# liuliu/ccv

Hardware: AMD Instinct MI355X
Metric: images/sec fwd+bwd VGG-D 224x224 bs256 (higher is better)
Workload: dtype f32 (Winograd-domain / fc GEMMs: exact bf16x3 split, all 9 products, fp32 accumulate); 1 GPU; VGG-D (ccv vgg_d_params, 225x225x3 crop, NHWC) forward+backward+SGD, batch 256 per GPU, random-init weights; global_batch=256, parallelism=dp1, conv_relu=convolution epilogue (NNC_MI355X_CONV_ALGO_FUSE_RELU)

## Files before the change

ccv_amd/csrc/cmd_conv.cpp:

```cpp
#include "gemm_launch.h"
#include "chan_sums.h"
#include "winograd.h"
#include "wino_fused.h"
#include "wino_wgrad_fused.h"
#include "conv_c3.h"
#include "conv_depthwise.h"

using namespace nnc;

namespace {

static size_t align256(size_t x) { return (x + 255) & ~(size_t)255; }

struct back_share_t {
	int want_v;
	int want_bits;
	int GYn, GXn, KB;
	float* v;
	unsigned* bits;
	size_t v_off, bits_off;
};

static void* g_dbg_bits_dst = 0;
static size_t g_dbg_bits_cap = 0, g_dbg_bits_got = 0;
static long g_back_shared[2] = { 0, 0 };

struct conv_geom_t {
	int N, H, W, C;
	int OH, OW, K;
	int kh, kw, Cg, Kg, groups;
	int sy, sx, pby, pbx, dy, dx;
};

struct conv_call_t {
	int relu_want, relu_done, mask_want, mask_done;
	Image4 mask;
	int staged;
	back_share_t share;
};
static bool mask_fits(const Image4& m, const Image4& dst)
// ... 159 lines not shown
	const long TH = (g.H + 3) / 4, TW = (g.W + 3) / 4;
	long most = 0;
	static const int shapes[3][2] = { { 4, 4 }, { 2, 8 }, { 8, 2 } };
	for (int i = 0; i < 3; i++) {
		const long cover = ((TH + shapes[i][0] - 1) / shapes[i][0]) * ((TW + shapes[i][1] - 1) / shapes[i][1]);
		if (cover > most) most = cover;
	}
	return (size_t)g.N * most * ((g.C + WF_KT - 1) / WF_KT) * 1024;
}

template <bool FLIP>
static int conv_wino_fused_run(conv_call_t& call, const char* name, const conv_geom_t& g, const wino_fused_plan_t& p, const Image4& src, const float* w, const float* bias, const Image4& dst, const int pad_y, const int pad_x, ccv_nnc_stream_context_t* const ctx)
{
	const back_share_t& share = call.share;
	size_t bits_bytes = FLIP && mask_fits(call.mask, dst) && (long)p.groups * p.KB <= 0x7fffffffL ? (size_t)p.groups * p.KB * 1024 : 0;
	bool have_bits = FLIP && bits_bytes && share.bits && p.GH == 2 && p.GYn == share.GYn && p.GXn == share.GXn && p.KB == share.KB && p.uf_bytes <= share.bits_off;
	float* UF = (float*)workspace_of(ctx, have_bits ? share.bits_off + bits_bytes : p.uf_bytes + bits_bytes);
	if (have_bits && (!UF || (unsigned*)((char*)UF + share.bits_off) != share.bits)) { have_bits = false; UF = (float*)workspace_of(ctx, p.uf_bytes + bits_bytes); }
	if (!UF && bits_bytes) { bits_bytes = 0; UF = (float*)workspace_of(ctx, p.uf_bytes); }
	if (!UF) return CCV_NNC_EXEC_OOM;
	hipStream_t stream = stream_of(ctx);
	unsigned* const bits = have_bits ? share.bits : (bits_bytes ? (unsigned*)((char*)UF + p.uf_bytes) : 0);
	if (have_bits) call.mask_done = 1;
	else if (bits) {
		const dim3 grid((unsigned)((long)p.groups * p.KB));
		const Image4& m = call.mask;
		if (p.GH == 4) hipLaunchKernelGGL(HIP_KERNEL_NAME(wino_mask_pack_kernel<4, 4>), grid, dim3(256), 0, stream, (const float*)m.p, m.sn, m.sh, m.sw, bits, dst.h, dst.w, dst.c, p.GYn, p.GXn, p.KB);
		else if (p.GH == 2) hipLaunchKernelGGL(HIP_KERNEL_NAME(wino_mask_pack_kernel<2, 8>), grid, dim3(256), 0, stream, (const float*)m.p, m.sn, m.sh, m.sw, bits, dst.h, dst.w, dst.c, p.GYn, p.GXn, p.KB);
		else hipLaunchKernelGGL(HIP_KERNEL_NAME(wino_mask_pack_kernel<8, 2>), grid, dim3(256), 0, stream, (const float*)m.p, m.sn, m.sh, m.sw, bits, dst.h, dst.w, dst.c, p.GYn, p.GXn, p.KB);
		HIP_ENFORCE(hipGetLastError());
		call.mask_done = 1;
	}
	if (bits && g_dbg_bits_dst) {
		g_dbg_bits_got = (size_t)p.groups * p.KB * 1024;
		HIP_ENFORCE(hipMemcpyAsync(g_dbg_bits_dst, bits, g_dbg_bits_got < g_dbg_bits_cap ? g_dbg_bits_got : g_dbg_bits_cap, hipMemcpyDeviceToHost, stream));
		HIP_ENFORCE(hipStreamSynchronize(stream));
		g_dbg_bits_dst = 0;
	}
// ... 89 lines not shown
	if (bits && (share.GYn * 2 != p.t.TH || share.GXn * 8 != p.t.TW || g.C % WF_KT)) {
		const int r = fill_f32((float*)bits, bits_bytes / sizeof(float), 0.f, ctx);
		if (r != CCV_NNC_EXEC_SUCCESS) return r;
	}
	for (int n0 = 0; n0 < g.N; n0 += nb) {
		const int ns = g.N - n0 < nb ? g.N - n0 : nb;
		const int T = ns * per_image;
		WinoTiles ti;
		ti.TH = p.t.TH; ti.TW = p.t.TW; ti.T = T;
		ti.H = a.h; ti.W = a.w; ti.sn = a.sn; ti.sh = a.sh; ti.sw = a.sw; ti.oy = -g.pby; ti.ox = -g.pbx; ti.C4 = g.C / 4;
		ti.d_c4.init(ti.C4); ti.d_tw.init(ti.TW); ti.d_th.init(ti.TH);
		if (bits) {
			WinoMaskOut mo;
			mo.bits = (unsigned char*)bits; mo.GYn = share.GYn; mo.GXn = share.GXn; mo.KB = share.KB;
			hipLaunchKernelGGL(HIP_KERNEL_NAME(wino_input_kernel<true>), dim3(blocks_exact((size_t)T * ti.C4, 256)), dim3(256), 0, stream, (const float*)a.p + (long)n0 * a.sn, V, ti, mo);
			share.bits = bits; share.bits_off = p.total();
			__atomic_fetch_add(&g_back_shared[1], 1L, __ATOMIC_RELAXED);
		} else hipLaunchKernelGGL(HIP_KERNEL_NAME(wino_input_kernel<false>), dim3(blocks_exact((size_t)T * ti.C4, 256)), dim3(256), 0, stream, (const float*)a.p + (long)n0 * a.sn, V, ti, WinoMaskOut());
		HIP_ENFORCE(hipGetLastError());
		ti.H = gr.h; ti.W = gr.w; ti.sn = gr.sn; ti.sh = gr.sh; ti.sw = gr.sw; ti.oy = 0; ti.ox = 0; ti.C4 = g.K / 4;
		ti.d_c4.init(ti.C4);
		const long blocks = ((long)T * (g.K / 4) + 255) / 256;
		const float* const grs = (const float*)gr.p + (long)n0 * gr.sn;
		if (Vg) {
			ti.oy = -1; ti.ox = -1;
			hipLaunchKernelGGL(wino_outgrad_both_kernel, dim3((unsigned)blocks), dim3(256), 0, stream, grs, Vg, W, ti, BP);
			share.v = Vg; share.v_off = p.total();
			__atomic_fetch_add(&g_back_shared[0], 1L, __ATOMIC_RELAXED);
		} else if (fuse_bias) hipLaunchKernelGGL(HIP_KERNEL_NAME(wino_outgrad_kernel<true>), dim3((unsigned)blocks), dim3(256), 0, stream, grs, W, ti, BP);
		else hipLaunchKernelGGL(HIP_KERNEL_NAME(wino_outgrad_kernel<false>), dim3((unsigned)blocks), dim3(256), 0, stream, grs, W, ti, (float*)0);
		HIP_ENFORCE(hipGetLastError());
// ... 44 lines not shown
	p->partial_bytes = (sizeof(float) * 36 * (size_t)s * g.K * g.C + 255) & ~(size_t)255;
	p->bias_bytes = (sizeof(float) * 4 * (size_t)s * g.K + 255) & ~(size_t)255;
	p->du_bytes = (sizeof(float) * 36 * (size_t)g.K * g.C + 255) & ~(size_t)255;
	return true;
}
static bool wino_wgrad_fused_images_ok(const Image4& a, const Image4& gr, const float* dw)
{
	const auto ok = [](const Image4& t) { return t.sc == 1 && aligned16(t.p) && t.sw % 4 == 0 && t.sh % 4 == 0 && (t.n == 1 || t.sn % 4 == 0) && ((long)(t.h - 1) * t.sh + (long)(t.w - 1) * t.sw + t.c) * 4 < 0x7ffff000L; };
	return ok(a) && ok(gr) && dw != 0;
}
static bool wino_wgrad_fused_preferred(const conv_geom_t& g)
{
	const long m = tune(TUNE_WINO_WGRAD_FUSED_MAX);
	return m > 0 && g.C <= m && g.K <= m;
}
static int conv_wino_wgrad_fused(const conv_geom_t& g, const wino_wgrad_fused_plan_t& p, const Image4& gr, const Image4& a, float* dw, float* dbias, bool* bias_done, const int flags, ccv_nnc_stream_context_t* const ctx)
{
	char* const ws = (char*)workspace_of(ctx, p.total());
	if (!ws) return CCV_NNC_EXEC_OOM;
	hipStream_t stream = stream_of(ctx);
	WinoWgradFusedArgs k;
	k.a = a.p; k.g = gr.p; k.partial = (float*)ws; k.bias_partial = dbias ? (float*)(ws + p.partial_bytes) : 0;
	k.a_sn = a.sn; k.a_sh = a.sh; k.a_sw = a.sw; k.g_sn = gr.sn; k.g_sh = gr.sh; k.g_sw = gr.sw;
	k.H = a.h; k.W = a.w; k.OH = gr.h; k.OW = gr.w; k.pad_y = g.pby; k.pad_x = g.pbx;
	k.GYn = p.GYn; k.GXn = p.GXn; k.groups = p.groups; k.C = g.C; k.K = g.K; k.kblocks = p.kblocks; k.cblocks = p.cblocks;
	k.slices = p.slices; k.per_slice = p.per_slice;
	k.a_image_bytes = (unsigned)(((long)(a.h - 1) * a.sh + (long)(a.w - 1) * a.sw + a.c) * 4);
	k.g_image_bytes = (unsigned)(((long)(gr.h - 1) * gr.sh + (long)(gr.w - 1) * gr.sw + gr.c) * 4);
	note_kernel("conv_wgrad_wino_fused");
	{
		const long T = (long)g.N * p.TH * p.TW;
		ProfScope prof("conv_wgrad_wino_fused|nnc::wino_wgrad_fused_kernel", 2.0 * 36.0 * (double)T * g.K * g.C, 0, g.K, g.C, (int)T, 36, p.slices, stream);
		hipLaunchKernelGGL(HIP_KERNEL_NAME(wino_wgrad_fused_kernel<0>), dim3((unsigned)(p.slices * p.kblocks * p.cblocks)), dim3(256), 0, stream, k);
		HIP_ENFORCE(hipGetLastError());
	}
	const long n = 36L * g.K * g.C;
	const int acc = (flags & CCV_NNC_ACCUMULATE_OUTPUT) ? 1 : 0;
	float* const dU = (float*)(ws + p.partial_bytes + p.bias_bytes);
	hipLaunchKernelGGL(wino_wgrad_fused_fold_kernel, dim3(blocks_exact((size_t)n, 256)), dim3(256), 0, stream, (const float*)k.partial, (const float*)k.bias_partial, dU, dbias, n, g.K, p.slices, acc);
	HIP_ENFORCE(hipGetLastError());
	hipLaunchKernelGGL(wino_wgrad_final_kernel, dim3(blocks_exact((size_t)g.K * g.C, 256)), dim3(256), 0, stream, (const float*)dU, dw, g.K, g.C, acc);
	HIP_ENFORCE(hipGetLastError());
	if (bias_done) *bias_done = dbias != 0;
	return CCV_NNC_EXEC_SUCCESS;
}

static bool wino_images_ok(const Image4& src, const Image4& dst, const float* w, const float* bias)
{
// ... 248 lines not shown
{
	return algo != CONV_ALGO_IMPLICIT_GEMM && wino_wgrad_plan(g, wp) && wino_images_ok(a, gr, dw, 0) && (algo >= CONV_ALGO_WINOGRAD || wino_preferred(wp->t, g.C, g.K));
}

static int conv_wgrad_nhwc(conv_call_t& call, const conv_geom_t& g, const Image4& gr, const Image4& a, float* dw, float* dbias, bool* bias_done, const int algo, const int flags, ccv_nnc_stream_context_t* const ctx)
{
	if (bias_done) *bias_done = false;
	if (a.sc != 1 || !pixel_linear(gr) || !image_fits_int(a)) return CCV_NNC_EXEC_INVALID;
	if (algo != CONV_ALGO_IMPLICIT_GEMM && conv_c3_ok(g, a, gr)) {
		const int r = conv_c3_wgrad(g, gr, a, dw, dbias, flags, ctx);
		if (r == CCV_NNC_EXEC_SUCCESS && bias_done) *bias_done = dbias != 0;
		if (r != CCV_NNC_EXEC_OOM) return r;
	}
	wino_wgrad_fused_plan_t wfp;
	if (conv_wgrad_takes_fused(g, gr, a, dw, algo, &wfp)) {
		const int r = conv_wino_wgrad_fused(g, wfp, gr, a, dw, dbias, bias_done, flags, ctx);
		if (r != CCV_NNC_EXEC_OOM) return r;
	}
	wino_wgrad_plan_t wp;
	if (conv_wgrad_takes_wino(g, gr, a, dw, algo, &wp)) {
		const int r = conv_wino_wgrad(call, g, wp, gr, a, dw, dbias, bias_done, flags, ctx);
		if (r != CCV_NNC_EXEC_OOM) return r;
	}
	const long P = (long)g.N * g.OH * g.OW;
	if (P > 0x7fffffffL) return CCV_NNC_EXEC_INVALID;
	const int NN = g.kh * g.kw * g.Cg;
	const bool vec = (g.Cg % 4 == 0) && (g.Kg % 4 == 0) && aligned16(a.p) && aligned16(gr.p) && a.sw % 4 == 0 && a.sh % 4 == 0 && (a.n == 1 || a.sn % 4 == 0) && gr.sw % 4 == 0;
	GemmOut out = { dw, (long)NN, 1, 0, 1.f, (flags & CCV_NNC_ACCUMULATE_OUTPUT) ? 1 : 0 };
	if (vec && conv_pointwise(g, a, gr)) {
		MatLoader<false, true> la, lb;
		la.p = gr.p; la.ldr = 1; la.ldk = gr.sw; la.R = g.K; la.K = (int)P;
// ... 438 lines not shown
	wino_wgrad_plan_t wgp;
	if (dw && cmd.algorithm != CONV_ALGO_IMPLICIT_GEMM && wino_wgrad_plan(g, &wgp) && wgp.total() > inner) inner = wgp.total();
	wino_wgrad_fused_plan_t wfgp;
	if (dw && cmd.algorithm != CONV_ALGO_IMPLICIT_GEMM && wino_wgrad_fused_plan(g, &wfgp) && wfgp.total() > inner) inner = wfgp.total();
	if (h && cmd.algorithm != CONV_ALGO_IMPLICIT_GEMM && wino_fused_scratch_bound(g.C, g.K) + wino_fused_mask_bound(call, g) > inner) inner = wino_fused_scratch_bound(g.C, g.K) + wino_fused_mask_bound(call, g);
	if (h && cmd.algorithm != CONV_ALGO_IMPLICIT_GEMM && conv_dgrad_parity_scratch(g) > inner) inner = conv_dgrad_parity_scratch(g);
	if (dw && cmd.algorithm != CONV_ALGO_IMPLICIT_GEMM && g.C == 3 && conv_c3_wgrad_scratch_bound(g.K) > inner) inner = conv_c3_wgrad_scratch_bound(g.K);
	back_share_t& share = call.share = back_share_t();
	const long share_on = tune(TUNE_CONV_BACK_SHARE);
	if (h && dw && a && w && share_on && !stage_io && !stage_w && g.pby == 1 && g.pbx == 1 && g.OH == g.H && g.OW == g.W && ai.sc == 1 && gi.sc == 1 && pixel_linear(gi) && pixel_linear(hi) && image_fits_int(ai) && image_fits_int(gi)
		&& !(cmd.algorithm != CONV_ALGO_IMPLICIT_GEMM && conv_c3_ok(g, ai, gi))) {
		wino_wgrad_fused_plan_t wf;
		wino_wgrad_plan_t wg;
		wino_fused_plan_t fp;
		wino_plan_t wp;
		if (!conv_wgrad_takes_fused(g, gi, ai, dw->data.f32, cmd.algorithm, &wf) && conv_wgrad_takes_wino(g, gi, ai, dw->data.f32, cmd.algorithm, &wg) && wino_slice_images(g.N, wg.t.TH * wg.t.TW, g.C, g.K) == g.N) {
			if (conv_dgrad_takes_fused(g, gi, hi, cmd.algorithm, &fp)) {
				if ((share_on & 2) && call.mask_want && fp.GH == 2 && mask_fits(ai, hi) && (long)fp.groups * fp.KB <= 0x7fffffffL && fp.uf_bytes <= wg.total()) {
					share.want_bits = 1; share.GYn = fp.GYn; share.GXn = fp.GXn; share.KB = fp.KB;
					if (wg.total() + (size_t)fp.groups * fp.KB * 1024 > inner) inner = wg.total() + (size_t)fp.groups * fp.KB * 1024;
				}
			} else if ((share_on & 1) && dbias && 256 % (g.K / 4) == 0 && conv_dgrad_takes_wino(g, gi, w->data.f32, hi, cmd.algorithm, &wp) && wp.TH == wg.t.TH && wp.TW == wg.t.TW && wp.u_bytes + wp.m_bytes <= wg.total()) {
				share.want_v = 1;
				if (wg.total() + wg.w_bytes > inner) inner = wg.total() + wg.w_bytes;
			}
		}
	}
	WorkspaceScope ws(stream_context, ng + na + nh + nw + ndw, inner);
	char* p = (char*)ws.prefix();
	if ((ng + na + nh + nw + ndw) && !p) return CCV_NNC_EXEC_OOM;
	int ret;
// ... 494 lines not shown
			const int ret = fwd ? _conv_forw(call, c, hint, trial_flags, inputs, input_size, outputs, output_size, stream_context) : _conv_back(call, c, hint, trial_flags, inputs, input_size, outputs, output_size, stream_context);
			HIP_ENFORCE(hipEventRecord(e1, stream));
			HIP_ENFORCE(hipEventSynchronize(e1));
			if (ret != CCV_NNC_EXEC_SUCCESS) ok = 0;
			else HIP_ENFORCE(hipEventElapsedTime(&ms, e0, e1));
		}
		if (ok && (!have_best || ms < best_ms)) { best = algo; best_ms = ms; have_best = 1; }
	}
	HIP_ENFORCE(hipEventDestroy(e0));
	HIP_ENFORCE(hipEventDestroy(e1));
	return best;
}

}

extern "C" long nnc_mi355x_debug_conv_back_shared(int what) { return what == 0 || what == 1 ? __atomic_load_n(&g_back_shared[what], __ATOMIC_RELAXED) : 0; }
extern "C" size_t nnc_mi355x_debug_conv_mask_bits(void* dst, size_t capacity)
{
	g_dbg_bits_dst = dst; g_dbg_bits_cap = capacity;
	return g_dbg_bits_got;
}

extern "C" void _register_command_CCV_NNC_CONVOLUTION_FORWARD_backend_CCV_NNC_BACKEND_GPU_CUDNN(ccv_nnc_cmd_backend_registry_t* const registry)
{
	registry->tensor_formats = CCV_TENSOR_FORMAT_NCHW | CCV_TENSOR_FORMAT_NHWC;
	registry->tensor_datatypes = CCV_32F | CCV_16F;
	registry->tensor_memory = CCV_TENSOR_GPU_MEMORY;
	registry->algorithms = CONV_ALGO_COUNT;
	registry->exec = _conv_forw_any;
	registry->autotune = _conv_autotune;
	NNC_DEPALETTIZED(registry, _conv_forw_any);
// ... 24 lines not shown
```

ccv_amd/csrc/device_rt.cpp:

```cpp
#include "common.h"
#include <atomic>
#include <pthread.h>
#include <dlfcn.h>
#include <vector>
#include <list>
#include <deque>
#include <mutex>
#include <unordered_map>

namespace {

struct device_local_t {
	hipStream_t stream;
	void* workspace;
	size_t workspace_size;
	int device;
	void* staging;
	size_t staging_size;
	void* palette;
	size_t palette_size;
	void* cluster_sync;
	unsigned cluster_epoch;
	unsigned long cluster_capture;
	unsigned long capture_alias;
// ... 91 lines not shown
	return l;
}

inline hipStream_t effective_stream(device_local_t* const l)
{
	if (g_capture_active.load(std::memory_order_acquire) > 0 && l->capture_alias == g_capture_id.load(std::memory_order_acquire) && l->capture_alias && l->device >= 0 && l->device < CAP_MAX_DEVICES && g_cap_rep[l->device]) return g_cap_rep[l->device];
	return l->stream;
}

}

namespace nnc {
int g_force_tile = 0;
int g_force_splits = 0;
static const char* const g_tune_names[TUNE_COUNT] = { "WINO_SLICE_KB", "WINO_FUSED_MAX_C", "WINO_FUSED_GRID", "GRID_WG_PER_CU", "WINO_WGRAD_FUSED_MAX", "GEMM_BUFFER_LOADS", "CONV_NCHW_HALF_F16", "BN_SMALL_PLANES", "SDPA_MFMA", "BN_CLUSTER", "GEMM_VEC_EPILOGUE", "POOL_ROWS", "GEMM_HALF_CHUNK8", "LSTM_PERSISTENT", "LSTM_ROWS", "GEMM_BF16X3", "BN_CLUSTER_SLOTS", "GEMM_BATCH_XCD", "CONV_BACK_SHARE", "CONV_DEPTHWISE", "ACT_HALF_NATIVE", "MUL_PLANES" };
static long g_tune_values[TUNE_COUNT] = { 0, 128, 0, 0, 128, 1, 32, 1, 1, 1, 1, 1, 1, 1, 1, 1, 0, 1, 3, 1, 1, 1 };
static int g_tune_env_read = 0;
long tune(int key)
{
	if (!g_tune_env_read) {
		for (int i = 0; i < TUNE_COUNT; i++) {
			char name[64];
			snprintf(name, sizeof(name), "NNC_MI355X_%s", g_tune_names[i]);
			const char* v = getenv(name);
			if (v && *v) g_tune_values[i] = atol(v);
		}
		g_tune_env_read = 1;
	}
	return key >= 0 && key < TUNE_COUNT ? g_tune_values[key] : 0;
}
}
// ... 1234 lines not shown
```

ccv_amd/csrc/isa.h:

```cpp
#pragma once
#include <hip/hip_runtime.h>

namespace nnc {

typedef float floatx16 __attribute__((ext_vector_type(16)));
typedef float floatx4 __attribute__((ext_vector_type(4)));
typedef _Float16 half_t;
typedef _Float16 halfx8 __attribute__((ext_vector_type(8)));
typedef _Float16 halfx4 __attribute__((ext_vector_type(4)));
typedef int wf_rsrc_t __attribute__((ext_vector_type(4)));
typedef unsigned int bf16x8_t __attribute__((ext_vector_type(4)));

#ifdef NNC_HIP_EMULATOR

#define NNC_PIN_V(x) ((void)0)
#define NNC_PIN_S(x) ((void)0)
#define WF_WAIT_VMCNT(n) __builtin_amdgcn_wave_barrier()
#define WF_MFMA(ACC, A, B, IN_AGPR) (ACC) = __builtin_amdgcn_mfma_f32_16x16x4f32((A), (B), (ACC), 0, 0, 0)
#define WF_MFMA0(ACC, A, B, IN_AGPR) (ACC) = __builtin_amdgcn_mfma_f32_16x16x4f32((A), (B), (floatx4{ 0.f, 0.f, 0.f, 0.f }), 0, 0, 0)
__device__ __forceinline__ wf_rsrc_t wf_make_rsrc(const void* base, unsigned bytes)
{
	const unsigned long long b = (unsigned long long)base;
	return wf_rsrc_t{ (int)(unsigned)b, (int)(unsigned)(b >> 32), (int)bytes, 0 };
}
__device__ __forceinline__ unsigned wf_lds_addr(float* p) { return (unsigned)(unsigned long long)p; }
__device__ __forceinline__ void wf_dma16(const wf_rsrc_t r, float* lds_base, unsigned lds_addr, unsigned voff, unsigned soff)
{
	const unsigned long long b = (unsigned long long)(unsigned)r[0] | (unsigned long long)(unsigned)r[1] << 32;
	float* const dst = (float*)((char*)lds_base + (lds_addr - wf_lds_addr(lds_base)));
// ... 20 lines not shown
#define NNC_PK_FMA_HI(acc, h, rp) do { (acc)[0] += (h)[0] * (rp)[1]; (acc)[1] += (h)[1] * (rp)[1]; } while (0)
#define NNC_WAIT_VM0_ONLY() ((void)0)
static inline float nnc_fast_exp2(const float x) { return exp2f(x); }
static inline float nnc_fast_rcp(const float x) { return 1.f / x; }
#define NNC_LAUNCH_CONCURRENT(kernel, grid, block, shmem, stream, ...) emuLaunchConcurrentKernel(kernel, grid, block, shmem, stream, __VA_ARGS__)
static inline unsigned nnc_fetch_add_agent(unsigned* p, unsigned v) { const unsigned o = *p; *p = o + v; return o; }
static inline void nnc_store_agent(unsigned* p, unsigned v) { *p = v; }
static inline void nnc_store_granule(unsigned long long* p, unsigned tag, float value) { unsigned u; memcpy(&u, &value, 4); *p = ((unsigned long long)tag << 32) | u; }
static inline unsigned long long nnc_load_granule(const unsigned long long* p) { return *(const volatile unsigned long long*)p; }
#define NNC_SPIN_SLEEP() emu::spin_yield()
static inline unsigned nnc_mul24(unsigned a, unsigned b) { return (a & 0xffffffu) * (b & 0xffffffu); }

#else

__device__ __forceinline__ unsigned nnc_mul24(unsigned a, unsigned b) { return __umul24(a, b); }

#define NNC_PIN_V(x) asm volatile("" : "+v"(x))
#define NNC_PIN_S(x) asm volatile("" : "+s"(x))
#define WF_WAIT_VMCNT(n) __builtin_amdgcn_s_waitcnt(((n) & 15) | (7 << 4) | (15 << 8) | (((n) >> 4) << 14))
#define WF_MFMA0(ACC, A, B, IN_AGPR) do { \
		if (IN_AGPR) asm volatile("v_mfma_f32_16x16x4_f32 %0, %1, %2, 0" : "+a"(ACC) : "v"(A), "v"(B)); \
		else asm volatile("v_mfma_f32_16x16x4_f32 %0, %1, %2, 0" : "+v"(ACC) : "v"(A), "v"(B)); \
	} while (0)
#define WF_MFMA(ACC, A, B, IN_AGPR) do { \
		if (IN_AGPR) asm volatile("v_mfma_f32_16x16x4_f32 %0, %1, %2, %0" : "+a"(ACC) : "v"(A), "v"(B)); \
		else asm volatile("v_mfma_f32_16x16x4_f32 %0, %1, %2, %0" : "+v"(ACC) : "v"(A), "v"(B)); \
	} while (0)
__device__ __forceinline__ wf_rsrc_t wf_make_rsrc(const void* base, unsigned bytes)
{
	const unsigned long long b = (unsigned long long)base;
// ... 53 lines not shown
```

ccv_amd/csrc/wino_fused.h:

```cpp
#pragma once
#include <utility>
#include "winograd.h"

namespace nnc {

constexpr int WF_KT = 32;
constexpr int WF_CC = 8;
constexpr int WF_U_FLOATS = 36 * 64 * 2 * 2;
constexpr int WF_HP = 352;
constexpr int WF_P_FLOATS = 2 * WF_HP * 4;
constexpr int WF_P_PIECES = 11;
constexpr int WF_Z_AGPR = 30;
constexpr unsigned WF_OOB = 0x7ffff000u;

template <class F, int... I> __device__ __forceinline__ void wf_static_for_impl(F&& f, std::integer_sequence<int, I...>) { (f(GroupId<I>()), ...); }
template <int N, class F> __device__ __forceinline__ void wf_static_for(F&& f) { wf_static_for_impl(f, std::make_integer_sequence<int, N>()); }

typedef float f2 __attribute__((ext_vector_type(2)));

template <int GH, int GW>
struct WfGeom {
	static constexpr int RH = 4 * GH + 2, RW = 4 * GW + 2, NPIX = RH * RW;
	static_assert(GH * GW == 16 && NPIX <= WF_HP, "tile group must be 16 tiles whose patch region fits the buffer");
	static constexpr __host__ __device__ int cy(int yy) { return GH + (yy < 2 ? 1 : 0); }
// ... 330 lines not shown
		const __amdgpu_buffer_rsrc_t rs_dst = __builtin_amdgcn_make_buffer_rsrc((void*)(a.dst + (long)it.n * a.d_sn), 0, a.dst_image_bytes, 0x00020000);
		const int kq = it.kb * WF_KT + (lane & 7) * 4;
		const bool kok = (it.live != 0) & (kq < a.K);
		float bv[4];
#pragma unroll
		for (int i = 0; i < 4; i++) bv[i] = (a.bias && kq < a.K) ? a.bias[kq + i] : 0.f;
		const int dh4 = (int)a.d_sh * 4, dw4 = (int)a.d_sw * 4;
		const wf_rsrc_t rs_item = wf_make_rsrc(a.dst + (long)it.n * a.d_sn, a.dst_image_bytes);
		const int base_y = it.gy * GH * 4, base_x = it.gx * GW * 4;
		const unsigned s_item = (unsigned)base_y * (unsigned)dh4 + (unsigned)base_x * (unsigned)dw4 + (unsigned)it.kb * (WF_KT * 4);
		const int hy0 = a.OH - base_y, hx0 = a.OW - base_x;
		const int ly = lane >> 5, lx = (lane >> 3) & 3;
		const unsigned lane_off_item = kok ? (unsigned)(ly * dh4 + lx * dw4 + (lane & 7) * 16) : WF_OOB;
		const float relu_lo = a.relu ? 0.f : -__builtin_inff();
		unsigned mb[4] = { ~0u, ~0u, ~0u, ~0u };
		if constexpr (MASK) {
			const unsigned* const mp = a.mask_bits + ((((long)it.n * a.GYn + it.gy) * a.GXn + it.gx) * a.KB + it.kb) * 256 + lane;
#pragma unroll
			for (int r = 0; r < 4; r++) mb[r] = it.live ? mp[r * 64] : 0u;
		}
#pragma unroll
		for (int r = 0; r < 4; r++) {
#pragma unroll
			for (int j = 0; j < 2; j++) {
				float s[4][6];
				if constexpr (DBG & 2048) {
#pragma unroll
					for (int i = 0; i < 4; i++)
#pragma unroll
						for (int jj = 0; jj < 4; jj++) st[g * TS + (i * 4 + jj) * 32 + j * 16 + ti] = acc[i * 4 + jj][j][r];
					continue;
// ... 5 lines not shown
					wino_at(col, y);
#pragma unroll
					for (int i = 0; i < 4; i++) s[i][zx] = y[i];
				}
#pragma unroll
				for (int i = 0; i < 4; i++) {
					float y[4];
					wino_at(s[i], y);
#pragma unroll
					for (int jj = 0; jj < 4; jj++) st[g * TS + (i * 4 + jj) * 32 + j * 16 + ti] = y[jj];
				}
			}
			__builtin_amdgcn_wave_barrier();
			if (r == 0) WF_WAIT_VMCNT(0);
			if constexpr (NEWST) {
#pragma unroll
				for (int e = 0; e < 8; e++) {
					const int tile = 4 * (e >> 1) + r;
					const int cy = (tile >> GWL) * 4 + (e & 1) * 2, cx = (tile & (GW - 1)) * 4;
					const float4 v = *(const float4*)(st + (e >> 1) * TS + ((e & 1) * 8 + (lane >> 3)) * 32 + (lane & 7) * 4);
					const unsigned soff = s_item + (unsigned)cy * (unsigned)dh4 + (unsigned)cx * (unsigned)dw4;
					const bool ok = (ly < hy0 - cy) & (lx < hx0 - cx);
					const unsigned voff = ok ? lane_off_item : WF_OOB;
					float o0 = wf_max(v.x + bv[0], relu_lo), o1 = wf_max(v.y + bv[1], relu_lo), o2 = wf_max(v.z + bv[2], relu_lo), o3 = wf_max(v.w + bv[3], relu_lo);
					if constexpr (MASK) {
						const unsigned m = mb[r] >> (4 * e);
						o0 = (m & 1) ? o0 : 0.f; o1 = (m & 2) ? o1 : 0.f; o2 = (m & 4) ? o2 : 0.f; o3 = (m & 8) ? o3 : 0.f;
					}
					if constexpr (DBG & 128) { NNC_PIN_V(o0); NNC_PIN_V(o1); NNC_PIN_V(o2); NNC_PIN_V(o3); }
					else wf_store16<ST_POLICY>(rs_item, voff, soff, o0, o1, o2, o3);
				}
			} else {
#pragma unroll
			for (int e = 0; e < 8; e++) {
				const int pid = e * 8 + (lane >> 3);
				const int gp = pid >> 4, px = pid & 15;
				const int tile = 4 * gp + r;
				const int oy = (it.gy * GH + (tile >> GWL)) * 4 + (px >> 2), ox = (it.gx * GW + (tile & (GW - 1))) * 4 + (px & 3);
				const float4 v = *(const float4*)(st + gp * TS + px * 32 + (lane & 7) * 4);
				const unsigned voff = (kok & (oy < a.OH) & (ox < a.OW)) ? (unsigned)(oy * dh4 + ox * dw4 + kq * 4) : WF_OOB;
// ... 88 lines not shown
```

ccv_amd/csrc/wino_wgrad_fused.h:

```cpp
#pragma once
#include "wino_fused.h"

namespace nnc {

typedef float f2v __attribute__((ext_vector_type(2)));

constexpr int WG_KB = 32, WG_CB = 64;
constexpr int WG_GH = 2, WG_GW = 4;
constexpr int WG_RH = 4 * WG_GH + 2, WG_RW = 4 * WG_GW + 2;
constexpr int WG_A_BYTES = WG_RH * WG_RW * WG_CB * 4;
constexpr int WG_G_BYTES = (4 * WG_GH) * (4 * WG_GW) * WG_KB * 4;
constexpr int WG_A_PIECES = WG_A_BYTES / 1024, WG_G_PIECES = WG_G_BYTES / 1024;
constexpr int WG_STAGE_BYTES = WG_A_BYTES + WG_G_BYTES;
static_assert(WG_A_BYTES % 1024 == 0 && WG_G_BYTES % 1024 == 0 && 2 * WG_STAGE_BYTES <= 160 * 1024, "two stages of whole DMA pieces in LDS");
constexpr int WG_A_PER_WAVE = (WG_A_PIECES + 3) / 4, WG_G_PER_WAVE = WG_G_PIECES / 4;
constexpr int WG_PIECES_PER_WAVE = WG_A_PER_WAVE + WG_G_PER_WAVE;

struct WinoWgradFusedArgs {
	const float* a;
	const float* g;
	float* partial;
	float* bias_partial;
	long a_sn, a_sh, a_sw, g_sn, g_sh, g_sw;
	int H, W, OH, OW;
	int pad_y, pad_x;
	int GYn, GXn;
	int groups;
	int C, K;
	int kblocks, cblocks;
	int slices;
	int per_slice;
	unsigned a_image_bytes, g_image_bytes;
};

template <int DBG = 0>
__global__ void __launch_bounds__(256, 1) wino_wgrad_fused_kernel(const WinoWgradFusedArgs p)
{
	__shared__ __attribute__((aligned(16))) float lds[2 * WG_STAGE_BYTES / 4 + 256];
	const int t = threadIdx.x, lane = t & 63;
	const int wave = __builtin_amdgcn_readfirstlane(t >> 6) & 3;
	const int wk = wave >> 1, wc = wave & 1;
	const int ch = lane & 15, slot = lane >> 4;
	const int nb = p.kblocks * p.cblocks;
	const int xcd = (int)blockIdx.x & 7, r = (int)blockIdx.x >> 3;
	const int slice = xcd * (p.slices >> 3) + r / nb, blk = r % nb;
	const int kb = blk / p.cblocks, cb = blk - kb * p.cblocks;
	int g_first = slice * p.per_slice, g_end = g_first + p.per_slice;
	if (g_end > p.groups) g_end = p.groups;
	const int gpi = p.GYn * p.GXn;

// ... 7 lines not shown
	int ayx[WG_A_PER_WAVE], gyx[WG_G_PER_WAVE];
#pragma unroll
	for (int i = 0; i < WG_A_PER_WAVE; i++) {
		const int q = wave + 4 * i, pi = q * 4 + (lane >> 4);
		ayx[i] = q < WG_A_PIECES ? ((pi / WG_RW) << 8 | (pi % WG_RW)) : 0xff00;
	}
#pragma unroll
	for (int i = 0; i < WG_G_PER_WAVE; i++) {
		const int pj = (wave + 4 * i) * 8 + (lane >> 3);
		gyx[i] = (pj / (4 * WG_GW)) << 8 | (pj % (4 * WG_GW));
	}
	const int a_coff = (cb * WG_CB + (lane & 15) * 4) * 4, g_coff = (kb * WG_KB + (lane & 7) * 4) * 4;
	const int a_sh4 = (int)p.a_sh * 4, a_sw4 = (int)p.a_sw * 4, g_sh4 = (int)p.g_sh * 4, g_sw4 = (int)p.g_sw * 4;
	const unsigned lds0 = __builtin_amdgcn_readfirstlane(wf_lds_addr(lds));
	wf_rsrc_t rs_a, rs_g;
	int aY0 = 0, aY1 = 0, aX0 = 0, aX1 = 0, gY1 = 0, gX1 = 0;
	auto set_group = [&](const int group) {
		const int n = group / gpi, gr = group - n * gpi;
		const int gy = gr / p.GXn, gx = gr - gy * p.GXn;
		const int ny0 = gy * 4 * WG_GH, nx0 = gx * 4 * WG_GW, nY0 = ny0 - p.pad_y, nX0 = nx0 - p.pad_x;
		rs_a = wf_make_rsrc(p.a + (long)n * p.a_sn + (long)nY0 * p.a_sh + (long)nX0 * p.a_sw, 0x7fff0000u);
		rs_g = wf_make_rsrc(p.g + (long)n * p.g_sn + (long)ny0 * p.g_sh + (long)nx0 * p.g_sw, 0x7fff0000u);
		aY0 = nY0 < 0 ? -nY0 : 0; aY1 = p.H - nY0 < WG_RH ? p.H - nY0 : WG_RH;
		aX0 = nX0 < 0 ? -nX0 : 0; aX1 = p.W - nX0 < WG_RW ? p.W - nX0 : WG_RW;
		gY1 = p.OH - ny0 < 4 * WG_GH ? p.OH - ny0 : 4 * WG_GH;
		gX1 = p.OW - nx0 < 4 * WG_GW ? p.OW - nx0 : 4 * WG_GW;
	};
	auto dma_piece = [&](auto ic, const int st, const bool live) {
		constexpr int i = decltype(ic)::value;
		if constexpr (i < WG_A_PER_WAVE) {
			const int Y = ayx[i] >> 8, X = ayx[i] & 255;
			const bool ok = live & (Y >= aY0) & (Y < aY1) & (X >= aX0) & (X < aX1);
			const unsigned voff = ok ? (unsigned)(Y * a_sh4 + X * a_sw4 + a_coff) : WF_OOB;
			const unsigned dst = wave + 4 * i < WG_A_PIECES ? lds0 + st * WG_STAGE_BYTES + (wave + 4 * i) * 1024 : lds0 + 2 * WG_STAGE_BYTES;
			wf_dma16(rs_a, lds, dst, voff, 0u);
		} else {
			constexpr int j = i - WG_A_PER_WAVE;
			const int y = gyx[j] >> 8, x = gyx[j] & 255;
			const bool ok = live & (y < gY1) & (x < gX1);
			const unsigned voff = ok ? (unsigned)(y * g_sh4 + x * g_sw4 + g_coff) : WF_OOB;
			wf_dma16(rs_g, lds, lds0 + st * WG_STAGE_BYTES + WG_A_BYTES + (wave + 4 * j) * 1024, voff, 0u);
		}
	};

	if (g_first < g_end) {
	set_group(g_first);
	NNC_ASM_NOPS("s_nop 4");
	wf_static_for<WG_PIECES_PER_WAVE>([&](auto nc) {
		constexpr int n = decltype(nc)::value, piece = n < 7 ? n : (n < 11 ? WG_A_PER_WAVE + (n - 7) : n - 4);
		dma_piece(GroupId<piece>(), 0, true);
	});

	for (int grp = g_first; grp < g_end; grp++) {
		const int st = (grp - g_first) & 1;
		if constexpr (!(DBG & 32)) {
			WF_WAIT_VMCNT(5);
			__builtin_amdgcn_s_barrier();
		}
		const bool has_next = grp + 1 < g_end;
		if (has_next) set_group(grp + 1);
		const float* const ab = lds + st * (WG_STAGE_BYTES / 4) + (4 * slot) * WG_CB + wc * 32 + 2 * ch;
		const float* const gb = lds + st * (WG_STAGE_BYTES / 4) + WG_A_BYTES / 4 + (4 * slot) * WG_KB + wk * 16 + ch;
		f2v W[36];
		if constexpr (DBG & 2) {
#pragma unroll
			for (int z = 0; z < 36; z++) W[z] = f2v{ 1.f + z, 2.f };
		} else {
			f2v e[4][4];
#pragma unroll
			for (int i = 0; i < 4; i++)
#pragma unroll
				for (int j = 0; j < 4; j++) e[i][j] = f2v{ gb[(i * (4 * WG_GW) + j) * WG_KB], gb[((4 + i) * (4 * WG_GW) + j) * WG_KB] };
// ... 56 lines not shown
				constexpr int mm = decltype(mc)::value, z = mm >> 1, jf = mm & 1;
				if constexpr (!(DBG & 16)) {
					if constexpr (ks == 0 && jf == 0) WF_MFMA(acc[z][0], W[z].x, V[z].x, z < WF_Z_AGPR);
					else if constexpr (ks == 0) WF_MFMA(acc[z][1], W[z].x, V[z].y, z < WF_Z_AGPR);
					else if constexpr (jf == 0) WF_MFMA(acc[z][0], W[z].y, V[z].x, z < WF_Z_AGPR);
					else WF_MFMA(acc[z][1], W[z].y, V[z].y, z < WF_Z_AGPR);
				}
				constexpr int m = ks * 72 + mm;
				if constexpr (m % 9 == 0 && !(DBG & 1)) {
					constexpr int n = m / 9;
					constexpr int piece = n < 7 ? n : (n < 11 ? WG_A_PER_WAVE + (n - 7) : n - 4);
					dma_piece(GroupId<piece>(), st ^ 1, has_next);
				}
			});
		});
	}
	}

	NNC_ASM_NOPS("s_nop 15\n\ts_nop 15");
	{
		float* const out = p.partial + (long)slice * 36 * p.K * p.C + (long)(kb * WG_KB + wk * 16 + 4 * slot) * p.C + cb * WG_CB + wc * 32 + 2 * ch;
		const long plane = (long)p.K * p.C;
#pragma unroll
		for (int z = 0; z < 36; z++)
#pragma unroll
			for (int j = 0; j < 2; j++)
#pragma unroll
				for (int i = 0; i < 4; i++) out[z * plane + (long)i * p.C + j] = acc[z][j][i];
		if (p.bias_partial && wc == 0 && cb == 0) p.bias_partial[((long)slice * 4 + slot) * p.K + kb * WG_KB + wk * 16 + ch] = bsum;
	}
// ... 24 lines not shown
```

Measured before the change: 3310 images/s.

## Emit ReLU mask bits from fused Winograd wgrad kernel for dgrad reuse

Result: no change. 3319 images/s, median of 5 (+0.3%).

```diff
diff --git a/ccv_amd/csrc/cmd_conv.cpp b/ccv_amd/csrc/cmd_conv.cpp
--- a/ccv_amd/csrc/cmd_conv.cpp
+++ b/ccv_amd/csrc/cmd_conv.cpp
@@ -15,15 +15,17 @@
 struct back_share_t {
 	int want_v;
 	int want_bits;
+	int want_bits_fused;
 	int GYn, GXn, KB;
 	float* v;
 	unsigned* bits;
+	int bits_gh;
 	size_t v_off, bits_off;
 };
 
 static void* g_dbg_bits_dst = 0;
 static size_t g_dbg_bits_cap = 0, g_dbg_bits_got = 0;
-static long g_back_shared[2] = { 0, 0 };
+static long g_back_shared[4] = { 0, 0, 0, 0 };
 
 struct conv_geom_t {
 	int N, H, W, C;
@@ -213,14 +215,14 @@
 {
 	const back_share_t& share = call.share;
 	size_t bits_bytes = FLIP && mask_fits(call.mask, dst) && (long)p.groups * p.KB <= 0x7fffffffL ? (size_t)p.groups * p.KB * 1024 : 0;
-	bool have_bits = FLIP && bits_bytes && share.bits && p.GH == 2 && p.GYn == share.GYn && p.GXn == share.GXn && p.KB == share.KB && p.uf_bytes <= share.bits_off;
+	bool have_bits = FLIP && bits_bytes && share.bits && p.GH == share.bits_gh && p.GYn == share.GYn && p.GXn == share.GXn && p.KB == share.KB && p.uf_bytes <= share.bits_off;
 	float* UF = (float*)workspace_of(ctx, have_bits ? share.bits_off + bits_bytes : p.uf_bytes + bits_bytes);
 	if (have_bits && (!UF || (unsigned*)((char*)UF + share.bits_off) != share.bits)) { have_bits = false; UF = (float*)workspace_of(ctx, p.uf_bytes + bits_bytes); }
 	if (!UF && bits_bytes) { bits_bytes = 0; UF = (float*)workspace_of(ctx, p.uf_bytes); }
 	if (!UF) return CCV_NNC_EXEC_OOM;
 	hipStream_t stream = stream_of(ctx);
 	unsigned* const bits = have_bits ? share.bits : (bits_bytes ? (unsigned*)((char*)UF + p.uf_bytes) : 0);
-	if (have_bits) call.mask_done = 1;
+	if (have_bits) { call.mask_done = 1; __atomic_fetch_add(&g_back_shared[3], 1L, __ATOMIC_RELAXED); }
 	else if (bits) {
 		const dim3 grid((unsigned)((long)p.groups * p.KB));
 		const Image4& m = call.mask;
@@ -340,7 +342,7 @@
 			WinoMaskOut mo;
 			mo.bits = (unsigned char*)bits; mo.GYn = share.GYn; mo.GXn = share.GXn; mo.KB = share.KB;
 			hipLaunchKernelGGL(HIP_KERNEL_NAME(wino_input_kernel<true>), dim3(blocks_exact((size_t)T * ti.C4, 256)), dim3(256), 0, stream, (const float*)a.p + (long)n0 * a.sn, V, ti, mo);
-			share.bits = bits; share.bits_off = p.total();
+			share.bits = bits; share.bits_off = p.total(); share.bits_gh = 2;
 			__atomic_fetch_add(&g_back_shared[1], 1L, __ATOMIC_RELAXED);
 		} else hipLaunchKernelGGL(HIP_KERNEL_NAME(wino_input_kernel<false>), dim3(blocks_exact((size_t)T * ti.C4, 256)), dim3(256), 0, stream, (const float*)a.p + (long)n0 * a.sn, V, ti, WinoMaskOut());
 		HIP_ENFORCE(hipGetLastError());
@@ -415,11 +417,18 @@
 	const long m = tune(TUNE_WINO_WGRAD_FUSED_MAX);
 	return m > 0 && g.C <= m && g.K <= m;
 }
-static int conv_wino_wgrad_fused(const conv_geom_t& g, const wino_wgrad_fused_plan_t& p, const Image4& gr, const Image4& a, float* dw, float* dbias, bool* bias_done, const int flags, ccv_nnc_stream_context_t* const ctx)
-{
-	char* const ws = (char*)workspace_of(ctx, p.total());
+static int conv_wino_wgrad_fused(conv_call_t& call, const conv_geom_t& g, const wino_wgrad_fused_plan_t& p, const Image4& gr, const Image4& a, float* dw, float* dbias, bool* bias_done, const int flags, ccv_nnc_stream_context_t* const ctx)
+{
+	back_share_t& share = call.share;
+	const size_t bits_bytes = share.want_bits_fused ? (size_t)g.N * share.GYn * share.GXn * share.KB * 1024 : 0;
+	char* const ws = (char*)workspace_of(ctx, p.total() + bits_bytes);
 	if (!ws) return CCV_NNC_EXEC_OOM;
 	hipStream_t stream = stream_of(ctx);
+	unsigned* const bits = bits_bytes ? (unsigned*)(ws + p.total()) : 0;
+	if (bits && (p.GYn & 1)) {
+		const int r = fill_f32((float*)bits, bits_bytes / sizeof(float), 0.f, ctx);
+		if (r != CCV_NNC_EXEC_SUCCESS) return r;
+	}
 	WinoWgradFusedArgs k;
 	k.a = a.p; k.g = gr.p; k.partial = (float*)ws; k.bias_partial = dbias ? (float*)(ws + p.partial_bytes) : 0;
 	k.a_sn = a.sn; k.a_sh = a.sh; k.a_sw = a.sw; k.g_sn = gr.sn; k.g_sh = gr.sh; k.g_sw = gr.sw;
@@ -428,11 +437,16 @@
 	k.slices = p.slices; k.per_slice = p.per_slice;
 	k.a_image_bytes = (unsigned)(((long)(a.h - 1) * a.sh + (long)(a.w - 1) * a.sw + a.c) * 4);
 	k.g_image_bytes = (unsigned)(((long)(gr.h - 1) * gr.sh + (long)(gr.w - 1) * gr.sw + gr.c) * 4);
+	k.mask_bits = (unsigned short*)bits;
 	note_kernel("conv_wgrad_wino_fused");
 	{
 		const long T = (long)g.N * p.TH * p.TW;
 		ProfScope prof("conv_wgrad_wino_fused|nnc::wino_wgrad_fused_kernel", 2.0 * 36.0 * (double)T * g.K * g.C, 0, g.K, g.C, (int)T, 36, p.slices, stream);
-		hipLaunchKernelGGL(HIP_KERNEL_NAME(wino_wgrad_fused_kernel<0>), dim3((unsigned)(p.slices * p.kblocks * p.cblocks)), dim3(256), 0, stream, k);
+		if (bits) {
+			hipLaunchKernelGGL(HIP_KERNEL_NAME(wino_wgrad_fused_kernel<0, true>), dim3((unsigned)(p.slices * p.kblocks * p.cblocks)), dim3(256), 0, stream, k);
+			share.bits = bits; share.bits_off = p.total(); share.bits_gh = 4;
+			__atomic_fetch_add(&g_back_shared[2], 1L, __ATOMIC_RELAXED);
+		} else hipLaunchKernelGGL(HIP_KERNEL_NAME(wino_wgrad_fused_kernel<0>), dim3((unsigned)(p.slices * p.kblocks * p.cblocks)), dim3(256), 0, stream, k);
 		HIP_ENFORCE(hipGetLastError());
 	}
 	const long n = 36L * g.K * g.C;
@@ -711,7 +725,7 @@
 	}
 	wino_wgrad_fused_plan_t wfp;
 	if (conv_wgrad_takes_fused(g, gr, a, dw, algo, &wfp)) {
-		const int r = conv_wino_wgrad_fused(g, wfp, gr, a, dw, dbias, bias_done, flags, ctx);
+		const int r = conv_wino_wgrad_fused(call, g, wfp, gr, a, dw, dbias, bias_done, flags, ctx);
 		if (r != CCV_NNC_EXEC_OOM) return r;
 	}
 	wino_wgrad_plan_t wp;
@@ -1180,7 +1194,13 @@
 		wino_wgrad_plan_t wg;
 		wino_fused_plan_t fp;
 		wino_plan_t wp;
-		if (!conv_wgrad_takes_fused(g, gi, ai, dw->data.f32, cmd.algorithm, &wf) && conv_wgrad_takes_wino(g, gi, ai, dw->data.f32, cmd.algorithm, &wg) && wino_slice_images(g.N, wg.t.TH * wg.t.TW, g.C, g.K) == g.N) {
+		if (conv_wgrad_takes_fused(g, gi, ai, dw->data.f32, cmd.algorithm, &wf)) {
+			if ((share_on & 4) && call.mask_want && conv_dgrad_takes_fused(g, gi, hi, cmd.algorithm, &fp) && fp.GH == 4 && fp.GW == 4 && mask_fits(ai, hi) && (long)fp.groups * fp.KB <= 0x7fffffffL
+				&& fp.uf_bytes <= wf.total() && fp.GXn == wf.GXn && fp.GYn == (wf.GYn + 1) / 2 && fp.KB == 2 * wf.cblocks && wf.kblocks >= 2) {
+				share.want_bits_fused = 1; share.GYn = fp.GYn; share.GXn = fp.GXn; share.KB = fp.KB;
+				if (wf.total() + (size_t)fp.groups * fp.KB * 1024 > inner) inner = wf.total() + (size_t)fp.groups * fp.KB * 1024;
+			}
+		} else if (conv_wgrad_takes_wino(g, gi, ai, dw->data.f32, cmd.algorithm, &wg) && wino_slice_images(g.N, wg.t.TH * wg.t.TW, g.C, g.K) == g.N) {
 			if (conv_dgrad_takes_fused(g, gi, hi, cmd.algorithm, &fp)) {
 				if ((share_on & 2) && call.mask_want && fp.GH == 2 && mask_fits(ai, hi) && (long)fp.groups * fp.KB <= 0x7fffffffL && fp.uf_bytes <= wg.total()) {
 					share.want_bits = 1; share.GYn = fp.GYn; share.GXn = fp.GXn; share.KB = fp.KB;
@@ -1705,7 +1725,7 @@
 
 }
 
-extern "C" long nnc_mi355x_debug_conv_back_shared(int what) { return what == 0 || what == 1 ? __atomic_load_n(&g_back_shared[what], __ATOMIC_RELAXED) : 0; }
+extern "C" long nnc_mi355x_debug_conv_back_shared(int what) { return what >= 0 && what <= 3 ? __atomic_load_n(&g_back_shared[what], __ATOMIC_RELAXED) : 0; }
 extern "C" size_t nnc_mi355x_debug_conv_mask_bits(void* dst, size_t capacity)
 {
 	g_dbg_bits_dst = dst; g_dbg_bits_cap = capacity;
diff --git a/ccv_amd/csrc/device_rt.cpp b/ccv_amd/csrc/device_rt.cpp
--- a/ccv_amd/csrc/device_rt.cpp
+++ b/ccv_amd/csrc/device_rt.cpp
@@ -129,7 +129,7 @@
 int g_force_tile = 0;
 int g_force_splits = 0;
 static const char* const g_tune_names[TUNE_COUNT] = { "WINO_SLICE_KB", "WINO_FUSED_MAX_C", "WINO_FUSED_GRID", "GRID_WG_PER_CU", "WINO_WGRAD_FUSED_MAX", "GEMM_BUFFER_LOADS", "CONV_NCHW_HALF_F16", "BN_SMALL_PLANES", "SDPA_MFMA", "BN_CLUSTER", "GEMM_VEC_EPILOGUE", "POOL_ROWS", "GEMM_HALF_CHUNK8", "LSTM_PERSISTENT", "LSTM_ROWS", "GEMM_BF16X3", "BN_CLUSTER_SLOTS", "GEMM_BATCH_XCD", "CONV_BACK_SHARE", "CONV_DEPTHWISE", "ACT_HALF_NATIVE", "MUL_PLANES" };
-static long g_tune_values[TUNE_COUNT] = { 0, 128, 0, 0, 128, 1, 32, 1, 1, 1, 1, 1, 1, 1, 1, 1, 0, 1, 3, 1, 1, 1 };
+static long g_tune_values[TUNE_COUNT] = { 0, 128, 0, 0, 128, 1, 32, 1, 1, 1, 1, 1, 1, 1, 1, 1, 0, 1, 7, 1, 1, 1 };
 static int g_tune_env_read = 0;
 long tune(int key)
 {
diff --git a/ccv_amd/csrc/isa.h b/ccv_amd/csrc/isa.h
--- a/ccv_amd/csrc/isa.h
+++ b/ccv_amd/csrc/isa.h
@@ -13,6 +13,8 @@
 
 #ifdef NNC_HIP_EMULATOR
 
+static inline int nnc_lane_fresh() { return (int)(threadIdx.x & 63); }
+static inline void nnc_shift_in_gt0(unsigned& acc, const float x) { acc = acc << 1 | (x > 0.f ? 1u : 0u); }
 #define NNC_PIN_V(x) ((void)0)
 #define NNC_PIN_S(x) ((void)0)
 #define WF_WAIT_VMCNT(n) __builtin_amdgcn_wave_barrier()
@@ -63,6 +65,8 @@
 #else
 
 __device__ __forceinline__ unsigned nnc_mul24(unsigned a, unsigned b) { return __umul24(a, b); }
+__device__ __forceinline__ int nnc_lane_fresh() { int r; asm volatile("v_mbcnt_lo_u32_b32 %0, -1, 0\n\tv_mbcnt_hi_u32_b32 %0, -1, %0" : "=v"(r)); return r; }
+__device__ __forceinline__ void nnc_shift_in_gt0(unsigned& acc, const float x) { asm("v_cmp_lt_f32_e32 vcc, 0, %1\n\tv_addc_co_u32_e32 %0, vcc, %0, %0, vcc" : "+v"(acc) : "v"(x) : "vcc"); }
 
 #define NNC_PIN_V(x) asm volatile("" : "+v"(x))
 #define NNC_PIN_S(x) asm volatile("" : "+s"(x))
diff --git a/ccv_amd/csrc/wino_fused.h b/ccv_amd/csrc/wino_fused.h
--- a/ccv_amd/csrc/wino_fused.h
+++ b/ccv_amd/csrc/wino_fused.h
@@ -368,7 +368,10 @@
 		const unsigned lane_off_item = kok ? (unsigned)(ly * dh4 + lx * dw4 + (lane & 7) * 16) : WF_OOB;
 		const float relu_lo = a.relu ? 0.f : -__builtin_inff();
 		unsigned mb[4] = { ~0u, ~0u, ~0u, ~0u };
-		if constexpr (MASK) {
+		if constexpr (MASK && (DBG & (1 << 17))) {
+#pragma unroll
+			for (int r = 0; r < 4; r++) NNC_PIN_V(mb[r]);
+		} else if constexpr (MASK) {
 			const unsigned* const mp = a.mask_bits + ((((long)it.n * a.GYn + it.gy) * a.GXn + it.gx) * a.KB + it.kb) * 256 + lane;
 #pragma unroll
 			for (int r = 0; r < 4; r++) mb[r] = it.live ? mp[r * 64] : 0u;
@@ -404,6 +407,7 @@
 			__builtin_amdgcn_wave_barrier();
 			if (r == 0) WF_WAIT_VMCNT(0);
 			if constexpr (NEWST) {
+				if constexpr (MASK && (DBG & (1 << 18))) NNC_PIN_V(mb[r]);
 #pragma unroll
 				for (int e = 0; e < 8; e++) {
 					const int tile = 4 * (e >> 1) + r;
@@ -413,7 +417,7 @@
 					const bool ok = (ly < hy0 - cy) & (lx < hx0 - cx);
 					const unsigned voff = ok ? lane_off_item : WF_OOB;
 					float o0 = wf_max(v.x + bv[0], relu_lo), o1 = wf_max(v.y + bv[1], relu_lo), o2 = wf_max(v.z + bv[2], relu_lo), o3 = wf_max(v.w + bv[3], relu_lo);
-					if constexpr (MASK) {
+					if constexpr (MASK && !(DBG & (1 << 18))) {
 						const unsigned m = mb[r] >> (4 * e);
 						o0 = (m & 1) ? o0 : 0.f; o1 = (m & 2) ? o1 : 0.f; o2 = (m & 4) ? o2 : 0.f; o3 = (m & 8) ? o3 : 0.f;
 					}
diff --git a/ccv_amd/csrc/wino_wgrad_fused.h b/ccv_amd/csrc/wino_wgrad_fused.h
--- a/ccv_amd/csrc/wino_wgrad_fused.h
+++ b/ccv_amd/csrc/wino_wgrad_fused.h
@@ -31,9 +31,10 @@
 	int slices;
 	int per_slice;
 	unsigned a_image_bytes, g_image_bytes;
+	unsigned short* mask_bits;
 };
 
-template <int DBG = 0>
+template <int DBG = 0, bool BITS = false>
 __global__ void __launch_bounds__(256, 1) wino_wgrad_fused_kernel(const WinoWgradFusedArgs p)
 {
 	__shared__ __attribute__((aligned(16))) float lds[2 * WG_STAGE_BYTES / 4 + 256];
@@ -71,6 +72,35 @@
 	const int a_sh4 = (int)p.a_sh * 4, a_sw4 = (int)p.a_sw * 4, g_sh4 = (int)p.g_sh * 4, g_sw4 = (int)p.g_sw * 4;
 	const unsigned lds0 = __builtin_amdgcn_readfirstlane(wf_lds_addr(lds));
 	wf_rsrc_t rs_a, rs_g;
+	const bool mb_on = BITS && kb < 2;
+	unsigned m_next = 0, m_prev = 0;
+	floatx4 m_px[4];
+	auto m_read = [&](const int st) {
+		const int l = nnc_lane_fresh();
+		const float* const mp = lds + st * (WG_STAGE_BYTES / 4) + (kb & 1) * 32 + ((1 + (l >> 5)) * WG_RW + 1 + 4 * wave + ((l >> 3) & 3)) * WG_CB + 4 * (l & 7);
+#pragma unroll
+		for (int e = 0; e < 4; e++) m_px[e] = *(const floatx4*)(mp + (2 * e * WG_RW) * WG_CB);
+	};
+	auto m_store = [&]() {
+		unsigned m = 0;
+		if constexpr (DBG & 256) {
+#pragma unroll
+			for (int e = 0; e < 4; e++) NNC_PIN_VEC(m_px[e]);
+			m = __builtin_bit_cast(unsigned, m_px[0][0]);
+		} else if constexpr (DBG & 128) {
+#pragma unroll
+			for (int e = 0; e < 4; e++)
+#pragma unroll
+				for (int i = 0; i < 4; i++) m |= (m_px[e][i] > 0.f ? 1u : 0u) << (4 * e + i);
+		} else {
+#pragma unroll
+			for (int e = 3; e >= 0; e--)
+#pragma unroll
+				for (int i = 3; i >= 0; i--) nnc_shift_in_gt0(m, m_px[e][i]);
+		}
+		if constexpr (DBG & 64) { NNC_PIN_V(m); return; }
+		p.mask_bits[((size_t)(m_prev >> 1) * 512 + (m_prev & 1)) + 2 * (wave * 64 + nnc_lane_fresh())] = (unsigned short)m;
+	};
 	int aY0 = 0, aY1 = 0, aX0 = 0, aX1 = 0, gY1 = 0, gX1 = 0;
 	auto set_group = [&](const int group) {
 		const int n = group / gpi, gr = group - n * gpi;
@@ -82,6 +112,7 @@
 		aX0 = nX0 < 0 ? -nX0 : 0; aX1 = p.W - nX0 < WG_RW ? p.W - nX0 : WG_RW;
 		gY1 = p.OH - ny0 < 4 * WG_GH ? p.OH - ny0 : 4 * WG_GH;
 		gX1 = p.OW - nx0 < 4 * WG_GW ? p.OW - nx0 : 4 * WG_GW;
+		if constexpr (BITS) m_next = (unsigned)(((n * ((p.GYn + 1) >> 1) + (gy >> 1)) * p.GXn + gx) * (2 * p.cblocks) + 2 * cb + (kb & 1)) * 2u + (unsigned)(gy & 1);
 	};
 	auto dma_piece = [&](auto ic, const int st, const bool live) {
 		constexpr int i = decltype(ic)::value;
@@ -112,7 +143,12 @@
 		const int st = (grp - g_first) & 1;
 		if constexpr (!(DBG & 32)) {
 			WF_WAIT_VMCNT(5);
+			if constexpr (BITS) NNC_WAIT_LGKM0();
 			__builtin_amdgcn_s_barrier();
+		}
+		if constexpr (BITS) {
+			if (mb_on && grp > g_first) m_store();
+			m_prev = m_next;
 		}
 		const bool has_next = grp + 1 < g_end;
 		if (has_next) set_group(grp + 1);
@@ -199,6 +235,10 @@
 				}
 			});
 		});
+		if constexpr (BITS) m_read(st);
+	}
+	if constexpr (BITS) {
+		if (mb_on) m_store();
 	}
 	}
 
```
